# locuslab/mpc.pytorch

Hardware: AMD Instinct MI355X
Metric: LQR problem-steps/sec (batch*T/s), n_state=12 n_ctrl=4 T=50 (higher is better)
Workload: dtype f32

## Files before the change

mpc.pytorch_amd/csrc/lqr_dpp16.hip:

```cpp
#include <string>
#include "lqr_common.h"

#define MPC_DEV __device__ __forceinline__
#define DPPM " row_mask:0xf bank_mask:0xf\n"

namespace mpclqr {
namespace wv {
typedef float f32x4 __attribute__((ext_vector_type(4)));
MPC_DEV int lane() { return (int)threadIdx.x; }
MPC_DEV int problem() { return (int)blockIdx.x; }
MPC_DEV unsigned long long clock() { return (unsigned long long)clock64(); }
MPC_DEV float rcp(float x) { return __builtin_amdgcn_rcpf(x); }
MPC_DEV void pin(float &x) { asm volatile("" : "+v"(x)); }
MPC_DEV bool uniform(bool c) { return c; }
MPC_DEV int uniform(int v) { return v; }
MPC_DEV bool any(bool c) { return __ballot(c) != 0ull; }
MPC_DEV unsigned long long ballot(bool c) { return __ballot(c); }
MPC_DEV float readlane(float x, int l) { return __int_as_float(__builtin_amdgcn_readlane(__float_as_int(x), __builtin_amdgcn_readfirstlane(l))); }
MPC_DEV double readlane_f64(double x, int l)
{
    const unsigned long long b = __double_as_longlong(x);
    const int ll = __builtin_amdgcn_readfirstlane(l);
    const unsigned lo = (unsigned)__builtin_amdgcn_readlane((int)(unsigned)b, ll), hi = (unsigned)__builtin_amdgcn_readlane((int)(unsigned)(b >> 32), ll);
    return __longlong_as_double(((unsigned long long)hi << 32) | lo);
// ... 259 lines not shown
        case 62: asm volatile("v_accvgpr_read_b32 %0, a248\n v_accvgpr_read_b32 %1, a249\n v_accvgpr_read_b32 %2, a250\n v_accvgpr_read_b32 %3, a251" : "=v"(r0), "=v"(r1), "=v"(r2), "=v"(r3)); break;
        case 63: asm volatile("v_accvgpr_read_b32 %0, a252\n v_accvgpr_read_b32 %1, a253\n v_accvgpr_read_b32 %2, a254\n v_accvgpr_read_b32 %3, a255" : "=v"(r0), "=v"(r1), "=v"(r2), "=v"(r3)); break;
    }
    return f32x4{r0, r1, r2, r3};
}

MPC_DEV double dpp_f64(double x, int) { return x; }
template <int CTRL> MPC_DEV double mov_dpp_f64(double x)
{
    const unsigned long long b = __double_as_longlong(x);
    const unsigned lo = (unsigned)__builtin_amdgcn_update_dpp(0, (int)(unsigned)b, CTRL, 0xf, 0xf, true);
    const unsigned hi = (unsigned)__builtin_amdgcn_update_dpp(0, (int)(unsigned)(b >> 32), CTRL, 0xf, 0xf, true);
    return __longlong_as_double(((unsigned long long)hi << 32) | lo);
}
MPC_DEV double row_sum_f64(double x)
{
    x += mov_dpp_f64<0xB1>(x);
    x += mov_dpp_f64<0x4E>(x);
    x += mov_dpp_f64<0x141>(x);
    x += mov_dpp_f64<0x140>(x);
    return x;
}

#ifndef MPC_DPP16_NSTAGE
#define MPC_DPP16_NSTAGE 4
#endif
#ifdef MPC_KF_LDS_BYTES
#define MPC_DPP16_LDS (MPC_KF_LDS_BYTES)
#else
#define MPC_DPP16_LDS (MPC_DPP16_NSTAGE * 9216)
#endif
#ifndef MPC_KKT16_NSTAGE
#define MPC_KKT16_NSTAGE 4
#endif
#if !defined(MPC_DPP16_WITH_KKT) && !defined(MPC_DPP16_NO_KKT) && MPC_DPP16_NSTAGE == 4
#define MPC_DPP16_WITH_KKT 1
#endif
__shared__ __attribute__((aligned(16))) char g_stage16[MPC_DPP16_LDS];
typedef __attribute__((address_space(3))) void lds_void_t;
typedef __attribute__((address_space(1))) const void glb_void_t;
#ifndef MPC_DPP16_C_AUX
#define MPC_DPP16_C_AUX 2
#endif
#ifndef MPC_DPP16_FR_AUX
#define MPC_DPP16_FR_AUX 0
#endif
MPC_DEV void store_out(float *g, float v)
{
#ifdef MPC_DPP16_OUT_CACHED
    *g = v;
#else
    __builtin_nontemporal_store(v, g);
#endif
}
#ifndef MPC_KKT_LD_AUX
#define MPC_KKT_LD_AUX 0
#endif
MPC_DEV void dma16_once(const void *g, unsigned off)
{
    __builtin_amdgcn_global_load_lds((glb_void_t *)g, (lds_void_t *)(g_stage16 + off), 16, 0, MPC_KKT_LD_AUX);
}
MPC_DEV void store_f32_out(float *g, float v) { *g = v; }
typedef float f32x2 __attribute__((ext_vector_type(2)));
MPC_DEV void store_f32x2_out(float *g, float a, float b)
{
#ifdef MPC_KF_CACHED_GRADS
    *(f32x2 *)g = f32x2{a, b};
#else
    __builtin_nontemporal_store(f32x2{a, b}, (f32x2 *)g);
#endif
}
MPC_DEV void store_f32_grad(float *g, float v)
{
#ifdef MPC_KF_CACHED_GRADS
    *g = v;
#else
    __builtin_nontemporal_store(v, g);
#endif
}
typedef float f32x4_a4 __attribute__((ext_vector_type(4), aligned(4)));
MPC_DEV void store_f32x4_grad(float *g, float __attribute__((ext_vector_type(4))) v)
{
#ifdef MPC_KF_CACHED_GRADS
    *(f32x4_a4 *)g = v;
#else
    __builtin_nontemporal_store(v, (f32x4_a4 *)g);
#endif
}
MPC_DEV float swap1(float x) { return __int_as_float(__builtin_amdgcn_update_dpp(0, __float_as_int(x), 0xB1, 0xf, 0xf, true)); }
MPC_DEV void dma16_if(bool active, const void *g, unsigned off)
{
    if (active) __builtin_amdgcn_global_load_lds((glb_void_t *)g, (lds_void_t *)(g_stage16 + off), 16, 0, 0);
}
template <int G> MPC_DEV void dma_buf(bool active, const void *base, unsigned nbytes, unsigned voff, unsigned off)
{
    static_assert(G == 4, "dword gathers");
    if (active) {
        __amdgpu_buffer_rsrc_t rs = __builtin_amdgcn_make_buffer_rsrc((void *)base, (short)0, (int)nbytes, 0x00020000);
        __builtin_amdgcn_raw_ptr_buffer_load_lds(rs, (lds_void_t *)(g_stage16 + off), 4, (int)voff, 0, 0, 0);
    }
}
MPC_DEV void dma4_if(bool active, const void *g, unsigned off)
{
    if (active) __builtin_amdgcn_global_load_lds((glb_void_t *)g, (lds_void_t *)(g_stage16 + off), 4, 0, 0);
}
template <int IMM, int BIAS> MPC_DEV void dma_buf_at(const void *base_biased, unsigned nbytes_biased, unsigned voff, unsigned anchor)
{
    static_assert(IMM >= 0 && IMM < 4096, "12-bit unsigned immediate");
    __amdgpu_buffer_rsrc_t rs = __builtin_amdgcn_make_buffer_rsrc((void *)base_biased, (short)0, (int)nbytes_biased, 0x00020000);
    __builtin_amdgcn_raw_ptr_buffer_load_lds(rs, (lds_void_t *)(g_stage16 + anchor), 4, (int)voff, 0, IMM, 0);
}
template <int IMM> MPC_DEV void dma4_at_if(bool active, const void *g, unsigned anchor)
{
    if (active) __builtin_amdgcn_global_load_lds((glb_void_t *)g, (lds_void_t *)(g_stage16 + anchor), 4, IMM, 0);
}
MPC_DEV void lds_store_f32x4(unsigned off, f32x4 v) { *(f32x4 *)(g_stage16 + off) = v; }
MPC_DEV void lds_store_f32(unsigned off, float v) { *(float *)(g_stage16 + off) = v; }
MPC_DEV void lds_sync() { asm volatile("" ::: "memory"); }
enum { DMA_PLAIN = 0, DMA_C = 1, DMA_LAST = 2 };
template <int IMM, int KIND = DMA_PLAIN> MPC_DEV void dma16_at(const void *g, unsigned mid)
{
    static_assert(IMM >= -4096 && IMM < 4096, "13-bit signed immediate");
    __builtin_amdgcn_global_load_lds((glb_void_t *)g, (lds_void_t *)(g_stage16 + mid), 16, IMM,
                                     KIND == DMA_C ? MPC_DPP16_C_AUX : (KIND == DMA_LAST ? MPC_DPP16_FR_AUX : 0));
}
template <int IMM> MPC_DEV void dma16_at_if(bool active, const void *g, unsigned mid)
{
    if (active) __builtin_amdgcn_global_load_lds((glb_void_t *)g, (lds_void_t *)(g_stage16 + mid), 16, IMM, 0);
}
MPC_DEV unsigned load_uniform_u32(const unsigned *g)
{
    typedef const __attribute__((address_space(4))) unsigned const_u32_t;
    return *(const_u32_t *)(unsigned long)g;
}
MPC_DEV float lds_f32(unsigned off) { return *(const float *)(g_stage16 + off); }
MPC_DEV float bits_f32(unsigned u) { return __uint_as_float(u); }
MPC_DEV unsigned f32_bits(float f) { return __float_as_uint(f); }
MPC_DEV f32x4 lds_f32x4(unsigned off) { return *(const f32x4 *)(g_stage16 + off); }
MPC_DEV void store_f32x4(float *g, f32x4 v) { *(f32x4 *)g = v; }
template <int N> MPC_DEV void dma_wait()
{
    static_assert(N >= 0 && N < 64, "vmcnt is 6 bits on gfx9");
    asm volatile("s_waitcnt vmcnt(%0) ; counted" ::"n"(N) : "memory");
}
MPC_DEV void fence_own_stores()
{
    __builtin_amdgcn_fence(__ATOMIC_RELEASE, "workgroup");
    __builtin_amdgcn_s_waitcnt(0);
    __builtin_amdgcn_fence(__ATOMIC_ACQUIRE, "workgroup");
}
}
}

#include "lqr_dpp16_body.h"

namespace mpclqr {
namespace {

template <int MODE>
__global__ void __launch_bounds__(64, 1) lqr_step_dpp16_kernel(StepParams<float> p)
{
    dpp16::step_wave<MODE>(p);
}

#if MPC_DPP16_NSTAGE == 4 || defined(MPC_DPP16_PAD_KKT)
static_assert((int)dpp16::KfP2<false>::SLOTS * (int)dpp16::KfP2<false>::STAGE + (int)dpp16::KfP2<false>::GST <= MPC_DPP16_LDS &&
              (int)dpp16::KfP2<false>::SLOTS >= 5, "the fused KKT kernel's second ring does not fit");
static_assert((int)dpp16::KfP2<true>::SLOTS * (int)dpp16::KfP2<true>::STAGE + (int)dpp16::KfP2<true>::GST <= MPC_DPP16_LDS &&
              (int)dpp16::KfP2<true>::SLOTS >= (dpp16::PADK ? 4 : 5), "the long-horizon fused KKT kernel's second ring does not fit");
static_assert((int)dpp16::LDS_TOTAL <= MPC_DPP16_LDS, "the fused KKT kernel's sweep ring does not fit");
template <bool MASKED>
__global__ void __launch_bounds__(64, 1) lqr_kkt_fused_dpp16_kernel(StepParams<float> p, dpp16::KktFusedArgs k)
{
    dpp16::kkt_fused_wave<MASKED>(p, k);
}
template <bool MASKED>
__global__ void __launch_bounds__(64, 1) lqr_kkt_fused_long_dpp16_kernel(StepParams<float> p, dpp16::KktFusedArgs k)
{
    dpp16::kkt_fused_wave<MASKED, true>(p, k);
}

#endif

#ifdef MPC_DPP16_WITH_KKT
static_assert(MPC_KKT16_NSTAGE * 8192 <= MPC_DPP16_LDS, "the KKT kernel's ring does not fit this compilation's staging array");
__global__ void __launch_bounds__(64, 1) lqr_kkt_dpp16_kernel(StepParams<float> p, dpp16::KktArgs k)
{
    dpp16::kkt_wave(p, k);
}

#endif
}

#ifdef MPC_DPP16_WITH_KKT
bool kkt_dpp16_supported(const StepParams<float> &p, const float *dx, const float *du, const float *dl_dx,
                         const float *dC, const float *dF)
{
    auto al = [](const void *q, long st, long sb) { return ((uintptr_t)q % 16 == 0) && (st % 4 == 0) && (sb % 4 == 0); };
    if (!(p.ns == 12 && p.nc == 4 && p.T >= 1)) return false;
    if (!al(p.C, p.C_st, p.C_sb) || !al(p.c, p.c_st, p.c_sb)) return false;
    if (p.T > 1 && !al(p.F, p.F_st, p.F_sb)) return false;
    return al(p.cur_x, 0, 0) && al(p.cur_u, 0, 0) && al(dx, 0, 0) && al(du, 0, 0) && al(dl_dx, 0, 0) && al(dC, 0, 0) &&
           (p.T == 1 || al(dF, 0, 0));
}

int launch_kkt_dpp16(const StepParams<float> &p, const float *dx, const float *du, const float *dl_dx, float *dC,
                     float *dc, float *dF, float *df, float *dx_init, hipStream_t st)
{
    dpp16::KktArgs k;
    k.dx = dx; k.du = du; k.dl_dx = dl_dx; k.dC = dC; k.dc = dc; k.dF = dF; k.df = df; k.dx_init = dx_init;
    hipLaunchKernelGGL(lqr_kkt_dpp16_kernel, dim3((p.B + 3) / 4), dim3(64), 0, st, p, k);
    hipError_t e = hipGetLastError();
    if (e != hipSuccess) {
        set_last_error((std::string("lqr_kkt_dpp16_kernel: ") + hipGetErrorString(e)).c_str());
        return MPC_E_LAUNCH;
    }
    return MPC_OK;
}

#endif

#ifdef MPC_DPP16_PAD_KKT
bool kkt_fused_dpp16_pad_supported(const StepParams<float> &p, const float *ws)
{
    return p.ns >= 1 && p.ns <= 12 && p.nc >= 1 && p.nc <= 4 && p.T >= 1 && (uintptr_t)ws % 16 == 0;
}
#define MPC_KF_LAUNCH launch_kkt_fused_dpp16_pad
#elif MPC_DPP16_NSTAGE == 4
#define MPC_KF_LAUNCH launch_kkt_fused_dpp16
bool kkt_fused_dpp16_supported(const StepParams<float> &p, const float *dl_dx, const float *dl_du, const float *dC,
                               const float *dF, const float *ws)
{
    auto al = [](const void *q, long st, long sb) { return ((uintptr_t)q % 16 == 0) && (st % 4 == 0) && (sb % 4 == 0); };
    if (!(p.ns == 12 && p.nc == 4 && p.T >= 1)) return false;
    if (!al(p.C, p.C_st, p.C_sb) || !al(p.c, p.c_st, p.c_sb)) return false;
    if (p.T > 1 && !al(p.F, p.F_st, p.F_sb)) return false;
    if (p.bound_mode == MPC_BOUND_TENSOR && (!al(p.lo, 0, 0) || !al(p.hi, 0, 0))) return false;
    return al(p.cur_x, 0, 0) && al(p.cur_u, 0, 0) && al(dl_dx, 0, 0) && al(dl_du, 0, 0) && al(dC, 0, 0) && al(ws, 0, 0) &&
           (p.T == 1 || al(dF, 0, 0));
}

int64_t kkt_fused_dpp16_workspace_bytes(int T, int B)
{
    return (int64_t)T * B * (dpp16::KF_VBLK + 24 + (T > dpp16::RG_STEPS ? 64 : 0)) * 4 + 64;
}
#endif

#if MPC_DPP16_NSTAGE == 4 || defined(MPC_DPP16_PAD_KKT)
int MPC_KF_LAUNCH(const StepParams<float> &p_in, const float *dl_dx, const float *dl_du, float *dC, float *dc, float *dF,
                  float *df, float *dx_init, float *dx_out, float *du_out, float *ws, float decay, int max_ls,
                  hipStream_t st)
{
    StepParams<float> p = p_in;
    p.zero_mask = nullptr;
    p.has_delta = 0;
    if (dpp16::PADK) p.c_symmetric = 1;
    dpp16::KktFusedArgs k;
    k.dl_dx = dl_dx; k.dl_du = dl_du; k.dC = dC; k.dc = dc; k.dF = dF; k.df = df; k.dx_init = dx_init;
    k.dx_out = dx_out; k.du_out = du_out; k.vws = ws; k.decay = decay; k.max_ls = max_ls;
    const dim3 grid((p.B + 3) / 4), block(64);
    if (p.T > dpp16::RG_STEPS) {
        if (p.bound_mode != MPC_BOUND_NONE) hipLaunchKernelGGL((lqr_kkt_fused_long_dpp16_kernel<true>), grid, block, 0, st, p, k);
        else hipLaunchKernelGGL((lqr_kkt_fused_long_dpp16_kernel<false>), grid, block, 0, st, p, k);
    } else if (p.bound_mode != MPC_BOUND_NONE) hipLaunchKernelGGL((lqr_kkt_fused_dpp16_kernel<true>), grid, block, 0, st, p, k);
    else hipLaunchKernelGGL((lqr_kkt_fused_dpp16_kernel<false>), grid, block, 0, st, p, k);
    hipError_t e = hipGetLastError();
    if (e != hipSuccess) {
        set_last_error((std::string("lqr_kkt_fused_dpp16_kernel: ") + hipGetErrorString(e)).c_str());
        return MPC_E_LAUNCH;
    }
    return MPC_OK;
}

#endif

#if MPC_DPP16_NSTAGE == 4
bool dpp16_supported(const StepParams<float> &p)
{
    auto al = [](const void *q, long st, long sb) { return ((uintptr_t)q % 16 == 0) && (st % 4 == 0) && (sb % 4 == 0); };
    if (!(p.ns == 12 && p.nc == 4 && p.T >= 1 && p.max_ls >= 1 && p.max_ls <= 16)) return false;
    if (!al(p.C, p.C_st, p.C_sb) || !al(p.c, p.c_st, p.c_sb)) return false;
    if (p.T > 1 && !al(p.F, p.F_st, p.F_sb)) return false;
    if (p.f && !al(p.f, p.f_st, p.f_sb)) return false;
    if (!al(p.cur_x, 0, 0) || !al(p.cur_u, 0, 0)) return false;
    if (p.bound_mode == MPC_BOUND_TENSOR && (!al(p.lo, 0, 0) || !al(p.hi, 0, 0))) return false;
    if (p.zero_mask && (uintptr_t)p.zero_mask % 4 != 0) return false;
    return true;
}

#endif

#ifndef MPC_DPP16_PAD_KKT
#ifdef MPC_DPP16_PAD
#define MPC_DPP16_LAUNCH launch_step_dpp16_pad
bool dpp16_pad_supported(const StepParams<float> &p)
{
    return p.ns >= 1 && p.ns <= 12 && p.nc >= 1 && p.nc <= 4 && p.T >= 1 && p.max_ls >= 1 && p.max_ls <= 16 && !p.env.kind;
}
#define MPC_DPP16_TAKES(p) dpp16_pad_supported(p)
#elif MPC_DPP16_NSTAGE == 4
#define MPC_DPP16_LAUNCH launch_step_dpp16
#else
#define MPC_DPP16_LAUNCH launch_step_dpp16_ring2
bool dpp16_supported(const StepParams<float> &p);
#endif
int MPC_DPP16_LAUNCH(const StepParams<float> &p, hipStream_t st)
// ... 24 lines not shown
```

mpc.pytorch_amd/csrc/lqr_dpp16_body.h:

```cpp
#pragma once
#include <math.h>
#include "lqr_params.h"
#include "lqr_small_math.h"

#ifndef MPC_STAT
#define MPC_STAT(i)
#endif

#ifndef MPC_DEVM
#define MPC_DEVM MPC_DEV
#endif

#ifndef MPC_DPP16_NSTAGE
#define MPC_DPP16_NSTAGE 4
#endif
#ifndef MPC_DPP16_QP_WARM
#define MPC_DPP16_QP_WARM 0
#endif

#ifdef MPC_DPP16_PAD
#define MPC_DPP16_PADK 1
#else
#define MPC_DPP16_PADK 0
#endif

namespace mpclqr {
namespace dpp16 {
constexpr bool PADK = MPC_DPP16_PADK != 0;
constexpr unsigned OOB_OFF = 0x7fff0000u;
enum { PAD_BIAS = 4096 };
MPC_DEV int pad_tau(int pj, int ns, int nc) { return pj < 12 ? (pj < ns ? pj : -1) : (pj - 12 < nc ? ns + (pj - 12) : -1); }

#ifdef MPC_DPP16_PROF
struct Prof { unsigned long long acc[16]; unsigned long long last; };
#define PROF_DECL Prof prof_; for (int i_ = 0; i_ < 16; ++i_) prof_.acc[i_] = 0; prof_.last = wv::clock()
#define PROF_ARG , Prof &prof_
#define PROF_PASS , prof_
#define PROF_MARK(slot) do { asm volatile("s_waitcnt lgkmcnt(0)" ::: "memory"); const unsigned long long n_ = wv::clock(); prof_.acc[slot] += n_ - prof_.last; prof_.last = n_; } while (0)
#define PROF_MARK_ALL(slot) do { asm volatile("s_waitcnt vmcnt(0) lgkmcnt(0)" ::: "memory"); const unsigned long long n_ = wv::clock(); prof_.acc[slot] += n_ - prof_.last; prof_.last = n_; } while (0)
#else
#define PROF_DECL
#define PROF_ARG
#define PROF_PASS
#define PROF_MARK(slot)
#define PROF_MARK_ALL(slot)
#endif

typedef StepParams<float> P;
using wv::f32x4;

constexpr bool con(int MODE) { return MODE == 1 || MODE == 2; }
constexpr bool rgm(int MODE) { return MODE < 1; }

enum { RG_STEPS = 64 };
template <bool ON> struct Gains {};
MPC_DEV void gain_put(Gains<true> &, int t, f32x4 v) { wv::rg_put(t, v); }
MPC_DEV f32x4 gain_get(const Gains<true> &, int t) { return wv::rg_get(t); }
MPC_DEV void gain_put(Gains<false> &, int, f32x4) {}
MPC_DEV f32x4 gain_get(const Gains<false> &, int) { return f32x4{0.f, 0.f, 0.f, 0.f}; }
using mfma16::Sym4;
using mfma16::Ldl4;
using mfma16::ldl4;
using mfma16::ldl4_solve;
using mfma16::eclampf;
using mfma16::sel;

struct Gj4 {
    float nl[4];
    float inv[4];
};
MPC_DEV void gj4_solve(const Gj4 &g, float (&z)[4])
{
#define MPC_GJ4_APPLY(c, a) wv::fmac_bcast_settled<4 * (a)>(z[a], g.nl[c], z[c])
    MPC_GJ4_APPLY(0, 1); MPC_GJ4_APPLY(0, 2); MPC_GJ4_APPLY(0, 3);
    MPC_GJ4_APPLY(1, 0); MPC_GJ4_APPLY(1, 2); MPC_GJ4_APPLY(1, 3);
    MPC_GJ4_APPLY(2, 0); MPC_GJ4_APPLY(2, 1); MPC_GJ4_APPLY(2, 3);
    MPC_GJ4_APPLY(3, 0); MPC_GJ4_APPLY(3, 1); MPC_GJ4_APPLY(3, 2);
#undef MPC_GJ4_APPLY
#pragma unroll
    for (int a = 0; a < 4; ++a) z[a] *= g.inv[a];
}
#ifdef MPC_DPP16_QP_LDL
using QpFac4 = Ldl4;
#else
using QpFac4 = Gj4;
#endif

MPC_DEV int pnqp4_rows(const Sym4 &s, const float q[4], const float lb[4], const float ub[4], int n_iter, int j,
                       float x[4], bool fr_out[4], QpFac4 &f, bool &converged)
{
    const float reg = 1e-11f;
    const float dg[4] = {s.s00 + reg - 1.f, s.s11 + reg - 1.f, s.s22 + reg - 1.f, s.s33 + reg - 1.f};
    const bool q0 = j < 4, q1 = j < 8, q2 = j < 12;
#define MPC_QV(v0, v1, v2, v3) (q0 ? (v0) : (q1 ? (v1) : (q2 ? (v2) : (v3))))
    const float Hc[4] = {MPC_QV(s.s00, s.s01, s.s02, s.s03), MPC_QV(s.s01, s.s11, s.s12, s.s13),
                         MPC_QV(s.s02, s.s12, s.s22, s.s23), MPC_QV(s.s03, s.s13, s.s23, s.s33)};
    const float lbv = MPC_QV(lb[0], lb[1], lb[2], lb[3]), ubv = MPC_QV(ub[0], ub[1], ub[2], ub[3]);
#ifndef MPC_DPP16_QP_LDL
    const float dgv = MPC_QV(dg[0], dg[1], dg[2], dg[3]);
    const bool qd[4] = {q0, q1 && !q0, q2 && !q1, !q2};
#endif
    float xv = MPC_QV(x[0], x[1], x[2], x[3]);
    float mv = -1.f;
    float done = 0.f, conv = 0.f, full = 0.f, it_ret = (float)(n_iter - 1);
#define MPC_HV(out, v) do { out = wv::bcast<0>(v) * Hc[0]; wv::fmac_bcast_settled<4>(out, v, Hc[1]); \
                            wv::fmac_bcast_settled<8>(out, v, Hc[2]); wv::fmac_bcast_settled<12>(out, v, Hc[3]); } while (0)
    float gv;
    MPC_HV(gv, xv);
    gv += MPC_QV(q[0], q[1], q[2], q[3]);
    MPC_STAT(4);
    for (int it = 0; it < n_iter; ++it) {
        if (done == 0.f) MPC_STAT(0);
        MPC_STAT(5);
        const float r_lo = (xv == lbv) ? gv : -1.f;
        const float r_hi = (xv == ubv) ? -gv : -1.f;
        const float mnv = (fmaxf(r_lo, r_hi) > 0.f) ? 0.f : 1.f;
        const float diff = wv::ring_sum(fabsf(mnv - mv));
        const bool confirmed = (diff == 0.f) & (full != 0.f) & (done == 0.f);
        it_ret = confirmed ? (float)it : it_ret;
        conv = confirmed ? 1.f : conv;
        done = confirmed ? 1.f : done;
        if (!wv::any(done == 0.f)) break;
        if (done == 0.f) MPC_STAT(1);
        MPC_STAT(6);
#ifdef MPC_DPP16_QP_LDL
        const float mn[4] = {wv::bcast<0>(mnv), wv::bcast<4>(mnv), wv::bcast<8>(mnv), wv::bcast<12>(mnv)};
        Ldl4 fn;
        {
            const float a10 = (mn[0] * mn[1]) * s.s01, a20 = (mn[0] * mn[2]) * s.s02, a30 = (mn[0] * mn[3]) * s.s03;
            const float a21 = (mn[1] * mn[2]) * s.s12, a31 = (mn[1] * mn[3]) * s.s13, a32 = (mn[2] * mn[3]) * s.s23;
            const float a00 = fmaf(mn[0], dg[0], 1.f), a11 = fmaf(mn[1], dg[1], 1.f);
            const float a22 = fmaf(mn[2], dg[2], 1.f), a33 = fmaf(mn[3], dg[3], 1.f);
            fn.i0 = wv::rcp(a00);
            fn.l10 = a10 * fn.i0; fn.l20 = a20 * fn.i0; fn.l30 = a30 * fn.i0;
            const float d1 = fmaf(-fn.l10, a10, a11);
            fn.i1 = wv::rcp(d1);
            const float t21 = fmaf(-fn.l20, a10, a21);
            const float t31 = fmaf(-fn.l30, a10, a31);
            fn.l21 = t21 * fn.i1; fn.l31 = t31 * fn.i1;
            const float d2 = fmaf(-fn.l21, t21, fmaf(-fn.l20, a20, a22));
            fn.i2 = wv::rcp(d2);
            const float t32 = fmaf(-fn.l31, t21, fmaf(-fn.l30, a20, a32));
            fn.l32 = t32 * fn.i2;
            const float d3 = fmaf(-fn.l32, t32, fmaf(-fn.l31, t31, fmaf(-fn.l30, a30, a33)));
            fn.i3 = wv::rcp(d3);
        }
        const float rv = mnv * gv;
        float y[4];
        ldl4_solve(fn, wv::bcast<0>(rv), wv::bcast<4>(rv), wv::bcast<8>(rv), wv::bcast<12>(rv), y);
        const float dxv = -(mnv * MPC_QV(y[0], y[1], y[2], y[3]));
#else
        Gj4 fn;
        float col[4];
#define MPC_GJ4_COL(c) do { col[c] = (mnv * wv::bcast<4 * (c)>(mnv)) * Hc[c]; col[c] = qd[c] ? dgq : col[c]; } while (0)
        const float dgq = fmaf(mnv, dgv, 1.f);
        MPC_GJ4_COL(0); MPC_GJ4_COL(1); MPC_GJ4_COL(2); MPC_GJ4_COL(3);
#undef MPC_GJ4_COL
        float sol = mnv * gv, invd = 0.f;
#define MPC_GJ4_PIVOT(c) do { const float inv = wv::rcp(wv::bcast<4 * (c)>(col[c])); fn.inv[c] = inv; \
                              const float t = -(col[c] * inv); fn.nl[c] = qd[c] ? 0.f : t; invd = qd[c] ? inv : invd; } while (0)
#define MPC_GJ4_ELIM(c, m) wv::fmac_bcast_settled<4 * (m)>(col[m], col[c], fn.nl[c])
#define MPC_GJ4_RHS(c) sol = fmaf(wv::bcast<4 * (c)>(sol), fn.nl[c], sol)
        MPC_GJ4_PIVOT(0); MPC_GJ4_ELIM(0, 1); MPC_GJ4_ELIM(0, 2); MPC_GJ4_ELIM(0, 3); MPC_GJ4_RHS(0);
        MPC_GJ4_PIVOT(1); MPC_GJ4_ELIM(1, 2); MPC_GJ4_ELIM(1, 3); MPC_GJ4_RHS(1);
        MPC_GJ4_PIVOT(2); MPC_GJ4_ELIM(2, 3); MPC_GJ4_RHS(2);
        MPC_GJ4_PIVOT(3); MPC_GJ4_RHS(3);
#undef MPC_GJ4_PIVOT
#undef MPC_GJ4_ELIM
#undef MPC_GJ4_RHS
        const float dxv = -(sol * invd);
#endif
        const float nrm2 = wv::ring_sum(dxv * dxv);
        f = fn;
        mv = mnv;
        const bool small = !(nrm2 >= 1e-8f) & (done == 0.f);
        it_ret = small ? (float)it : it_ret;
        conv = small ? 1.f : conv;
        done = small ? 1.f : done;
        const float live = 1.f - done;
        const float xnv = xv + dxv;
        float xcv = eclampf(xnv, lbv, ubv);
        const float out = wv::ring_sum(fabsf(xcv - xnv));
        float dv = (xcv - xv) * live, hdv;
        MPC_HV(hdv, dv);
        const bool inside = out == 0.f;
        full = inside ? 1.f : 0.f;
        const bool test = !inside & (done == 0.f);
        if (wv::any(test)) {
            if (test) MPC_STAT(2);
            const float den = wv::ring_sum(-gv * dv), dhd = wv::ring_sum(dv * hdv);
            const float arm = fmaf(-0.5f, dhd, den) * wv::rcp(den);
            bool go = test & (arm <= 0.1f);
            if (wv::any(go)) {
                float alpha = 0.1f;
                for (int count = 1; count < 10; ++count) {
                    if (go) MPC_STAT(3);
                    const float xt = eclampf(fmaf(alpha, dxv, xv), lbv, ubv);
                    const float dt = xt - xv;
                    float hdt;
                    MPC_HV(hdt, dt);
                    const float den2 = wv::ring_sum(-gv * dt), dhd2 = wv::ring_sum(dt * hdt);
                    const float arm2 = fmaf(-0.5f, dhd2, den2) * wv::rcp(den2);
                    xcv = go ? xt : xcv;
                    dv = go ? dt : dv;
                    hdv = go ? hdt : hdv;
// ... 895 lines not shown
    if (rgm(MODE)) {
        const float mult = L.j == 12 ? alpha : dx;
        un = s.tb + wv::quad_sums(s.rec[0] * mult, s.rec[1] * mult, s.rec[2] * mult, s.rec[3] * mult, L.j);
    } else {
        un = fmaf(alpha, s.kk, s.tb);
        wv::dot_bcast12(un, dx, s.Kr);
    }
    const float pre = un;
    if (con(MODE) && s.zm) un = 0.f;
    if (MODE == 2) {
        const float dlt = p.has_delta ? p.delta_u : 3.0e38f;
        const float l = fmaxf(s.lo, s.tb - dlt), h = fminf(s.hi, s.tb + dlt);
        un = eclampf(un, l, h);
    }
    e = L.isu ? (un - pre) + (alpha - 1.f) * s.kk : 0.f;
    return un;
}

template <int MODE, bool DIRECT>
MPC_DEV float stage_price(const Lane &L, const RoStage &s, float tp, float e, float dx)
{
    if (DIRECT) {
        float sq = 0.f;
        wv::dot_bcast16(sq, tp, s.Cr);
        return tp * fmaf(0.5f, sq, s.cj);
    }
    float se = 0.f;
    wv::dot_bcast_u4(se, e, s.Sr);
    const float quad = L.isu ? e * (0.5f * se) : 0.f;
    if (!con(MODE)) return quad;
    float w = 0.f;
    wv::dot_bcast_u4(w, e, s.Mc);
    const float mult = L.j < 12 ? dx : 1.f;
    return L.j <= 12 ? fmaf(mult, w, quad) : quad;
}

template <int MODE, bool DIRECT, bool CHECK, bool PAIR = false>
MPC_DEV void rollout_step(const P &p, const Lane &L, const RoStage &s, RoState &st, int t, Feed<MODE, true, DIRECT> &feed)
{
    const bool last = (t == p.T - 1);
    feed.template part<0>();
    float e, dx;
    const float un = control_law<MODE>(p, L, s, st.xs, st.alpha, e, dx);
    const float tp = L.isu ? un : st.xs;
    feed.template part<1>();
    if (DIRECT || !rgm(MODE) || st.price_on) st.cost += stage_price<MODE, DIRECT>(L, s, tp, e, dx);
    {
        const float d = sel(L.isu, s.tb - un, 0.f);
        st.du2 = fmaf(d, d, st.du2);
    }
    if (!PADK || L.ovalid) wv::store_out(st.out, tp);
    st.out += L.ostep;
    feed.template part<2>();
    if (!DIRECT && CHECK) {
        if (t > 0) {
            float r = fabsf(st.pred - s.tb) - 1e-5f * (1.f + fabsf(s.tb));
            r = (r == r) ? r : 1.f;
            r = sel(L.isu, 0.f, r);
            st.viol = r > st.viol ? r : st.viol;
        }
        if (!last) {
            float pn = s.fj;
            wv::dot_bcast16(pn, s.tb, s.Fr);
            st.pred = pn;
        }
    }
    feed.template part<3>();
    if (!last) {
        float xn = s.fj;
        wv::dot_bcast16(xn, tp, s.Fr);
        st.xs = xn;
    }
    if (PAIR) {
        float e1, dx1;
        const float un1 = control_law<MODE>(p, L, s, st.xs1, p.ls_decay, e1, dx1);
        const float tp1 = L.isu ? un1 : st.xs1;
        st.cost1 += stage_price<MODE, DIRECT>(L, s, tp1, e1, dx1);
        {
            const float d = sel(L.isu, s.tb - un1, 0.f);
            st.du21 = fmaf(d, d, st.du21);
        }
        *st.out1 = tp1;
        st.out1 += L.ostep1;
        if (!last) {
            float xn = s.fj;
            wv::dot_bcast16(xn, tp1, s.Fr);
            st.xs1 = xn;
        }
    }
}

enum { MAX_TRIALS = 15 };
struct Trials {
    float xs[MAX_TRIALS], cost[MAX_TRIALS], alpha[MAX_TRIALS];
    float du2_last;
    float *park;
    bool park_row;
    int park_k;
};

template <int MODE, bool DIRECT>
MPC_DEV void trials_step(const P &p, const Lane &L, const RoStage &s, Trials &tr, int nt, int t)
{
    const bool last = (t == p.T - 1);
    constexpr bool PARK = MODE == 2 && !DIRECT;
#pragma unroll
    for (int k = 0; k < MAX_TRIALS; ++k) {
        if (k < nt) {
            float e, dx;
            const float un = control_law<MODE>(p, L, s, tr.xs[k], tr.alpha[k], e, dx);
            const float tp = L.isu ? un : tr.xs[k];
            tr.cost[k] += stage_price<MODE, DIRECT>(L, s, tp, e, dx);
            if (PARK && k == tr.park_k) {
                const float d = sel(L.isu, s.tb - un, 0.f);
                tr.du2_last = fmaf(d, d, tr.du2_last);
                if (tr.park_row) *tr.park = tp;
                tr.park += L.ostep1;
            }
            if (!last) {
                float xn = s.fj;
                wv::dot_bcast16(xn, tp, s.Fr);
                tr.xs[k] = xn;
            }
        }
    }
}

template <int MODE, bool MULTI, bool DIRECT, bool CHECK, bool PAIR = false>
MPC_DEV void rollout_pass(const P &p, const Lane &L, Dma &d, int wave, const Gains<rgm(MODE)> &G, RoState &st, Trials &tr, int nt, double base PROF_ARG)
{
    const int T = p.T;
    float x0 = L.isu ? 0.f : (PADK ? (L.ovalid ? p.x_init[(long)L.pb * p.ns + L.j] : 0.f) : p.x_init[(long)L.pb * 12 + L.j]);
    wv::pin(x0);
    if (MULTI) {
#pragma unroll
        for (int k = 0; k < MAX_TRIALS; ++k) { tr.xs[k] = x0; tr.cost[k] = 0.f; }
        tr.du2_last = 0.f;
        tr.park = L.scr0;
    } else {
        st.xs = x0;
        st.cost = 0.f;
        st.du2 = 0.f;
        st.pred = 0.f;
        st.out = L.out0;
        if (PAIR) {
            st.xs1 = x0;
            st.cost1 = 0.f;
            st.du21 = 0.f;
            st.out1 = L.scr0;
        }
    }
    st.price_on = MULTI || wv::any(st.alpha != 1.f);
    const bool use_zm = con(MODE) && p.zero_mask != nullptr;
    enum { NS = RollRing<MODE, DIRECT>::SLOTS, LA = NS - 1, ND = RollDma<MODE, DIRECT>::N };
    static_assert((LA - 1) * ND + 2 * LA < 64, "vmcnt is 6 bits");
    unsigned zq[NS];
#pragma unroll
    for (int i = 0; i < NS; ++i) zq[i] = 0u;
    dma_seek<MODE, true, DIRECT>(d, p, L, wave);
    pad_clear(L.lane);
#pragma unroll
    for (int i = 0; i < LA; ++i) {
        if (i < T) {
            stage_issue<MODE, true, DIRECT>(d, stage_mid<MODE, true, DIRECT>(i));
            stage_move<MODE, true, DIRECT>(d, i + 1 <= T - 2);
            if (use_zm) zq[i] = zm_pick(L, zm_fetch(p, L, i));
        }
    }
    for (int t0 = 0; t0 < T; t0 += NS) {
#pragma unroll
        for (int i = 0; i < NS; ++i) {
            const int t = t0 + i;
            if (t < T) {
                PROF_MARK(7);
                if (T - 1 - t >= LA - 1) wv::dma_wait<(LA - 1) * ND>();
                else tail_wait<(LA >= 2 ? LA - 2 : 0), ND>(T - 1 - t);
                PROF_MARK(4);
                RoStage s;
                ro_read<MODE, DIRECT>(s, p, L, t, i, zq[i]);
                if (rgm(MODE)) {
                    s.rec = gain_get(G, t);
                    if (!DIRECT && st.price_on) rg_price_terms(s, L);
                }
                PROF_MARK(5);
                const int tn = t + LA;
                ZmRaw zr = {{0u, 0u, 0u, 0u}};
                if (use_zm && tn < T) zr = zm_fetch(p, L, tn);
                Feed<MODE, true, DIRECT> feed = {d, stage_mid<MODE, true, DIRECT>((i + LA) % NS), tn < T, tn + 1 <= T - 2};
                PROF_MARK(6);
                if (MULTI) {
                    feed.template part<0>(); feed.template part<1>(); feed.template part<2>(); feed.template part<3>();
                    trials_step<MODE, DIRECT>(p, L, s, tr, nt, t);
                } else {
                    rollout_step<MODE, DIRECT, CHECK, PAIR>(p, L, s, st, t, feed);
                }
                if (use_zm) zq[(i + LA) % NS] = zm_pick(L, zr);
            }
        }
    }
    wv::dma_wait<0>();
    if (MULTI) {
#pragma unroll
        for (int k = 0; k < MAX_TRIALS; ++k)
            if (k < nt) tr.cost[k] = (float)(base + (double)wv::row_sum(tr.cost[k]));
        tr.du2_last = wv::row_sum(tr.du2_last);
    } else {
        st.cost = (float)(base + (double)wv::row_sum(st.cost));
        st.du2 = wv::row_sum(st.du2);
        if (PAIR) {
            st.cost1 = (float)(base + (double)wv::row_sum(st.cost1));
            st.du21 = wv::row_sum(st.du21);
        }
    }
}

MPC_DEV Lane lane_as_slot(const Lane &L, int ps, const P &p, int wave)
{
    Lane X = L;
    const int dp = ps - L.p;
    const int pb = 4 * wave + ps < p.B ? 4 * wave + ps : p.B - 1;
    X.p = ps;
    X.pb = pb;
#pragma unroll
    for (int q = 0; q < 4; ++q) X.aFq[q] += dp * 768;
    X.aRec += dp * 256; X.aRecA += dp * 256; X.aRecF += dp * 256;
    X.aKrow += dp * 256; X.aMcol += dp * 256; X.aGcol += dp * 256; X.aFm += dp * 256;
#pragma unroll
    for (int b = 0; b < 4; ++b) X.aS[b] += dp * 256;
    X.scr0 = p.Kk + (long)p.T * p.B * 128 + (long)pb * 16 + L.j;
    return X;
}

template <int MODE, bool DIRECT, bool CHECK>
MPC_DEV void line_search(const P &p, const Lane &L, Dma &d, int wave, const Gains<rgm(MODE)> &G, RoState &rs, float old_cost, double base, float &full2 PROF_ARG)
{
    Trials tr;
    rs.alpha = 1.f;
    bool worse0 = false;
    bool copy_parked = false;
    if (MODE == 2 && !DIRECT && p.max_ls >= 2) {
        rollout_pass<MODE, false, DIRECT, CHECK, true>(p, L, d, wave, G, rs, tr, 0, base PROF_PASS);
        full2 = rs.du2;
        worse0 = rs.cost > old_cost;
        if (!wv::any(worse0)) return;
        const bool worse1 = worse0 && rs.cost1 > old_cost && p.max_ls > 2;
        if (worse0) {
            rs.alpha = p.ls_decay;
            rs.cost = rs.cost1;
            rs.du2 = rs.du21;
        }
        if (wv::any(worse1)) {
            const int nt = p.max_ls - 2;
            bool ended_on_last = false;
            const unsigned long long wm = wv::ballot(worse1 && L.j == 0);
            const int n_w = (int)__builtin_popcountll(wm);
            const bool shared = n_w == 1 && nt >= 4;
            const int ps1 = (int)(__builtin_ctzll(wm | (1ull << 63)) >> 4);
            const int nt_row = shared ? (nt + 3) / 4 : nt;
            const int r_last = shared ? (nt - 1) / nt_row : 0;
            if (shared) MPC_STAT(7); else MPC_STAT(8);
            {
                const int ps = ps1;
                const Lane X = lane_as_slot(L, shared ? ps : L.p, p, wave);
                const int idx0 = shared ? L.p * nt_row : 0;
                float a = p.ls_decay;
                for (int i = 0; i <= (idx0 < nt - 1 ? idx0 : nt - 1); ++i) a *= p.ls_decay;
#pragma unroll
                for (int k = 0; k < MAX_TRIALS; ++k) {
                    tr.alpha[k] = a;
                    if (idx0 + k + 1 <= nt - 1) a *= p.ls_decay;
                }
                tr.park_k = shared ? (L.p == r_last ? (nt - 1) - r_last * nt_row : -1) : nt - 1;
                tr.park_row = shared || worse1;
                const double base_s = shared ? wv::readlane_f64(base, 16 * ps) : base;
                const float old_s = shared ? wv::readlane(old_cost, 16 * ps) : old_cost;
                rollout_pass<MODE, true, DIRECT, CHECK>(p, X, d, wave, G, rs, tr, nt_row, base_s PROF_PASS);
                float acc = 0.f, cacc = 0.f, du2_l = tr.du2_last;
                int kacc = 0;
                bool found = false;
                if (shared) {
#pragma unroll
                    for (int r = 0; r < 4; ++r) {
#pragma unroll
                        for (int k = 0; k < MAX_TRIALS; ++k) {
                            if (k < nt_row && r * nt_row + k < nt && !found) {
                                acc = wv::readlane(tr.alpha[k], 16 * r);
                                cacc = wv::readlane(tr.cost[k], 16 * r);
                                kacc = r * nt_row + k;
                                if (!(cacc > old_s)) found = true;
                            }
                        }
                    }
                    du2_l = wv::readlane(tr.du2_last, 16 * r_last);
                } else {
#pragma unroll
                    for (int k = 0; k < MAX_TRIALS; ++k) {
                        if (k < nt && !found) {
                            acc = tr.alpha[k];
                            cacc = tr.cost[k];
                            kacc = k;
                            if (!(tr.cost[k] > old_cost)) found = true;
                        }
                    }
                }
                if (shared ? L.p == ps : worse1) {
                    rs.alpha = acc;
                    ended_on_last = kacc == nt - 1;
                    if (ended_on_last) { rs.cost = cacc; rs.du2 = du2_l; }
                }
            }
            if (wv::any(worse1 && !ended_on_last)) {
                rollout_pass<MODE, false, DIRECT, CHECK>(p, L, d, wave, G, rs, tr, 0, base PROF_PASS);
                return;
            }
        }
        copy_parked = true;
    }
    if (copy_parked) {
        PROF_MARK_ALL(9);
        wv::fence_own_stores();
        enum { COPY_N = 16 };
        const float *src = L.scr0;
        float *dst = L.out0;
        const int T = p.T;
        for (int t0 = 0; t0 < T; t0 += COPY_N) {
            float v[COPY_N];
#pragma unroll
            for (int i = 0; i < COPY_N; ++i) {
                const int t = t0 + i < T ? t0 + i : T - 1;
                v[i] = src[(long)t * L.ostep1];
            }
#pragma unroll
            for (int i = 0; i < COPY_N; ++i) {
                const int t = t0 + i < T ? t0 + i : T - 1;
                if (worse0 && (!PADK || L.ovalid)) wv::store_out(dst + (long)t * L.ostep, v[i]);
            }
        }
        PROF_MARK_ALL(12);
        return;
    }
#pragma unroll 1
    for (int phase = 0; phase < 3; ++phase) {
        rollout_pass<MODE, false, DIRECT, CHECK>(p, L, d, wave, G, rs, tr, 0, base PROF_PASS);
        if (phase == 0) {
            full2 = rs.du2;
            worse0 = rs.cost > old_cost && p.max_ls > 1;
            if (!wv::any(worse0)) break;
            if (worse0) rs.alpha = p.ls_decay;
        } else if (phase == 1) {
            const bool worse1 = worse0 && rs.cost > old_cost && p.max_ls > 2;
            if (!wv::any(worse1)) break;
            const int nt = p.max_ls - 2;
            float a = p.ls_decay;
#pragma unroll
            for (int k = 0; k < MAX_TRIALS; ++k) { a *= p.ls_decay; tr.alpha[k] = a; }
            rollout_pass<MODE, true, DIRECT, CHECK>(p, L, d, wave, G, rs, tr, nt, base PROF_PASS);
            if (worse1) {
                float acc = tr.alpha[0];
                bool found = false;
#pragma unroll
                for (int k = 0; k < MAX_TRIALS; ++k) {
                    if (k < nt && !found) {
                        acc = tr.alpha[k];
                        if (!(tr.cost[k] > old_cost)) found = true;
                    }
                }
                rs.alpha = acc;
            }
        }
    }
}

template <int MODE>
MPC_DEV void step_wave(const P &p)
{
    const int lane = wv::lane();
    const int wave = wv::problem();
    if (4 * wave >= p.B) return;
    Lane L;
    lane_init(L, lane, wave, p.B, !p.c_symmetric);
    L.out0 = L.isu ? p.new_u + (long)L.pb * 4 + L.a : p.new_x + (long)L.pb * 12 + L.j;
    L.ostep = L.isu ? (long)p.B * 4 : (long)p.B * 12;
    if (PADK) {
        L.ovalid = L.isu ? L.a < p.nc : L.j < p.ns;
#pragma unroll
        for (int a = 0; a < 4; ++a) L.padd[a] = (L.j == 12 + a && a >= p.nc) ? 1.f : 0.f;
        L.out0 = L.isu ? p.new_u + (long)L.pb * p.nc + (L.ovalid ? L.a : 0) : p.new_x + (long)L.pb * p.ns + (L.ovalid ? L.j : 0);
        L.ostep = L.isu ? (long)p.B * p.nc : (long)p.B * p.ns;
    }
    L.scr0 = p.Kk + (long)p.T * p.B * 128 + (long)L.pb * 16 + L.j;
    L.ostep1 = (long)p.B * 16;
    const int T = p.T;
    Dma d;
    Gains<rgm(MODE)> G;
    PROF_DECL;

    SwState ss;
#pragma unroll
    for (int i = 0; i < 12; ++i) ss.Vc[i] = 0.f;
    ss.vv = 0.f;
    ss.oc = 0.0;
    ss.w0 = 0.0;
    ss.warm = 0;
    ss.qp_total = 0;
    ss.status = 0;
    ss.asym = 0.f;
    ss.cmax = 0.f;
    ss.kprev[0] = ss.kprev[1] = ss.kprev[2] = ss.kprev[3] = 0.f;
    ss.rec_step = (long)p.B * 64;
    ss.rec = p.Kk + ((long)(T - 1) * p.B + L.pb) * 64 + 4 * L.j;
    ss.rec2_step = (long)p.B * 4;
    ss.rec2 = p.Kk + (long)T * p.B * 64 + ((long)(T - 1) * p.B + L.pb) * 4;
    {
        unsigned zq[NSTAGE] = {};
        dma_seek<MODE, false, false>(d, p, L, wave);
        pad_clear(L.lane);
#pragma unroll
        for (int i = 0; i < AHEAD; ++i) {
            const int ti = T - 1 - i;
            if (ti >= 0) {
                stage_issue<MODE, false, false>(d, stage_mid<MODE, false, false>(i));
                stage_move<MODE, false, false>(d, ti <= T - 2);
                if (MODE == 1) zq[i] = zm_pick(L, zm_fetch(p, L, ti));
            }
        }
        for (int k0 = 0; k0 < T; k0 += NSTAGE) {
#pragma unroll
            for (int i = 0; i < NSTAGE; ++i) {
                const int t = T - 1 - (k0 + i);
                if (t >= 0) {
                    PROF_MARK(3);
                    if (t >= AHEAD - 1) wv::dma_wait<(AHEAD - 1) * DMA_SWEEP>();
                    else wv::dma_wait<0>();
                    PROF_MARK(0);
                    SwStage s;
                    sw_read<MODE>(s, p, L, t, i, zq[i], ss.asym, ss.cmax);
                    PROF_MARK(1);
                    ZmRaw zr = {{0u, 0u, 0u, 0u}};
                    if (MODE == 1 && t >= AHEAD) zr = zm_fetch(p, L, t - AHEAD);
                    Feed<MODE, false, false> feed = {d, stage_mid<MODE, false, false>((i + AHEAD) % NSTAGE), t >= AHEAD, true};
                    PROF_MARK(2);
                    sweep_step<MODE>(p, L, s, ss, t, feed, G PROF_PASS);
                    if (MODE == 1) zq[(i + AHEAD) % NSTAGE] = zm_pick(L, zr);
                }
            }
        }
        wv::dma_wait<0>();
    }
    PROF_MARK_ALL(8);
    const double old_cost_d = wv::row_sum_f64(ss.oc);
    const float old_cost = (float)old_cost_d;
    if (!p.c_symmetric) ss.status |= MPC_ST_C_TESTED | (wv::row_max(ss.asym) > 1e-5f * wv::row_max(ss.cmax) ? (int)MPC_ST_C_ASYMMETRIC : 0);

    if (p.sweep_only) {
        if (L.j == 0) {
            if (p.old_costs) p.old_costs[L.pb] = old_cost;
            if (p.qp_iters) p.qp_iters[L.pb] = ss.qp_total;
            if (p.status) p.status[L.pb] = ss.status;
        }
        return;
    }
    wv::fence_own_stores();

    RoState rs;
    rs.viol = 0.f;
    float full2 = 0.f;
    if (p.on_dynamics) {
        line_search<MODE, false, false>(p, L, d, wave, G, rs, old_cost, old_cost_d + ss.w0, full2 PROF_PASS);
    } else {
        line_search<MODE, false, true>(p, L, d, wave, G, rs, old_cost, old_cost_d + ss.w0, full2 PROF_PASS);
        const bool off = wv::row_sum(rs.viol > 0.f ? 1.f : 0.f) > 0.f;
        const bool broken = off || (MODE == 2 && (ss.status & MPC_ST_PNQP_UNCONVERGED) != 0);
        if (wv::any(broken)) line_search<MODE, true, false>(p, L, d, wave, G, rs, old_cost, 0.0, full2 PROF_PASS);
        if (off) ss.status |= MPC_ST_NOMINAL_OFF_DYNAMICS;
    }
#ifdef MPC_DPP16_PROF
    PROF_MARK_ALL(9);
    if (p.K != nullptr && lane == 0)
        for (int i_ = 0; i_ < 16; ++i_) p.K[(long)wave * 16 + i_] = (float)prof_.acc[i_];
#endif
    int status = ss.status;
    if (!(rs.cost == rs.cost) || fabsf(rs.cost) > 3e38f) status |= MPC_ST_NONFINITE;
    if (L.j == 0) {
        const int b = L.pb;
        if (p.costs) p.costs[b] = rs.cost;
        if (p.old_costs) p.old_costs[b] = old_cost;
        if (p.full_du_norm) p.full_du_norm[b] = sqrtf(full2);
        if (p.alpha_du_norm) p.alpha_du_norm[b] = sqrtf(rs.du2);
        if (p.alphas) p.alphas[b] = rs.alpha;
        if (p.qp_iters) p.qp_iters[b] = ss.qp_total;
        if (p.status) p.status[b] = status;
    }
}


struct KktArgs {
    const float *dx, *du, *dl_dx;
    float *dC, *dc, *dF, *df, *dx_init;
};

#ifndef MPC_KKT16_NSTAGE
#define MPC_KKT16_NSTAGE 4
#endif
enum { K_c = 0, K_tau = 64, K_dtau = 128, K_rx = 192, KKT_STAGE = 8192, DMA_KKT = 8, KKT_NSTAGE = MPC_KKT16_NSTAGE,
       KKT_AHEAD = KKT_NSTAGE - 1 };

struct KktDma {
    const char *c_ptr[4];
    const char *f_ptr[3];
    const char *r_ptr;
    long c_step, f_step, r_step;
    bool r_active;
};

MPC_DEV void kkt_dma_init(KktDma &d, const P &p, const KktArgs &k, const Lane &L, int wave)
{
    const long B = p.B;
#pragma unroll
    for (int q = 0; q < 4; ++q) {
        const int pbk = 4 * wave + q < p.B ? 4 * wave + q : p.B - 1;
        d.c_ptr[q] = (const char *)(p.C + (long)pbk * p.C_sb) + 16 * src_granule_C(L.lane, 0);
    }
    d.c_step = 4 * p.C_st;
#pragma unroll
    for (int q = 0; q < 3; ++q) {
        const int G = 64 * q + L.lane;
        const int slot = G / 48, gi = G - 48 * slot;
        const int pbk = 4 * wave + slot < p.B ? 4 * wave + slot : p.B - 1;
        d.f_ptr[q] = p.T > 1 ? (const char *)(p.F + (long)pbk * p.F_sb) + 16 * src_granule_cols(gi, slot) : (const char *)p.C;
    }
    d.f_step = 4 * p.F_st;
    const int gi = L.lane & 15;
    const long pb = L.pb;
    d.r_active = gi < 15;
    const char *q = (const char *)p.c;
    long st = 0;
    if (gi < 4) { q = (const char *)(p.c + pb * p.c_sb + 4 * gi); st = 4 * p.c_st; }
    else if (gi < 7) { q = (const char *)(p.cur_x + pb * 12 + 4 * (gi - 4)); st = 4 * B * 12; }
    else if (gi == 7) { q = (const char *)(p.cur_u + pb * 4); st = 4 * B * 4; }
    else if (gi < 11) { q = (const char *)(k.dx + pb * 12 + 4 * (gi - 8)); st = 4 * B * 12; }
    else if (gi == 11) { q = (const char *)(k.du + pb * 4); st = 4 * B * 4; }
    else if (gi < 15) { q = (const char *)(k.dl_dx + pb * 12 + 4 * (gi - 12)); st = 4 * B * 12; }
    d.r_ptr = q;
    d.r_step = st;
}

MPC_DEV void kkt_stage_issue(const P &p, const KktDma &d, int t, int slot)
{
    const unsigned base = (unsigned)slot * KKT_STAGE;
    const long tl = t;
    const long tf = t < p.T - 1 ? t : (p.T > 1 ? p.T - 2 : 0);
#pragma unroll
    for (int q = 0; q < 4; ++q) wv::dma16_once(d.c_ptr[q] + tl * d.c_step, base + SC + 1024 * q);
#pragma unroll
    for (int q = 0; q < 3; ++q) wv::dma16_once(d.f_ptr[q] + (p.T > 1 ? tf * d.f_step : 0), base + SF + 1024 * q);
    wv::dma16_if(d.r_active, d.r_ptr + tl * d.r_step, base + SR);
}

MPC_DEV void kkt_wave(const P &p, const KktArgs &k)
{
    const int lane = wv::lane();
    const int wave = wv::problem();
    if (4 * wave >= p.B) return;
    Lane L;
    lane_init(L, lane, wave, p.B, false);
    const int T = p.T;
    KktDma d;
    kkt_dma_init(d, p, k, L, wave);
    float lam = 0.f, dlam = 0.f;
#pragma unroll
    for (int i = 0; i < KKT_AHEAD; ++i) kkt_stage_issue(p, d, T - 1 - i >= 0 ? T - 1 - i : 0, i);
    for (int k0 = 0; k0 < T; k0 += KKT_NSTAGE) {
#pragma unroll
        for (int i = 0; i < KKT_NSTAGE; ++i) {
            const int t = T - 1 - (k0 + i);
            if (t >= 0) {
                wv::dma_wait<(KKT_AHEAD - 1) * DMA_KKT>();
                const unsigned base = (unsigned)i * KKT_STAGE;
                float Cr[16], Fc[12];
#pragma unroll
                for (int q = 0; q < 4; ++q) {
                    const f32x4 v = wv::lds_f32x4(base + L.aCq[q]);
                    Cr[4 * q] = v[0]; Cr[4 * q + 1] = v[1]; Cr[4 * q + 2] = v[2]; Cr[4 * q + 3] = v[3];
                }
                const bool have = t < T - 1;
                if (have) {
#pragma unroll
                    for (int m = 0; m < 12; ++m) Fc[m] = wv::lds_f32(base + ((m & 1) ? L.aFo : L.aFe) + 64 * m);
                } else {
#pragma unroll
                    for (int m = 0; m < 12; ++m) Fc[m] = 0.f;
                }
                const float cj = wv::lds_f32(base + L.aRec + K_c);
                const float tj = wv::lds_f32(base + L.aRec + K_tau);
                const float dj = wv::lds_f32(base + L.aRec + K_dtau);
                const float rj = wv::lds_f32(base + SR + L.p * 256 + K_rx + 4 * (L.j < 12 ? L.j : 11));
// ... 608 lines not shown
```

Before: 2.248 billion.

## Software-pipeline LDS stage reads one step ahead in sweep and rollout loops

Adds a double-buffered register stage so the LDS reads for step t±1 are issued before computing step t, in both the backward sweep and the forward rollout, for unconstrained non-padded modes. The DMA lookahead is restructured so the whole ring is in flight (LA = NSTAGE) while waits use one fewer slot, and an explicit LDS drain waitcnt is inserted per step. The aim is to hide LDS read latency behind the previous step's math. The cost is extra register pressure, and the rollout ring is capped at four slots in regularised modes.

```diff
diff --git a/mpc.pytorch_amd/csrc/lqr_dpp16.hip b/mpc.pytorch_amd/csrc/lqr_dpp16.hip
--- a/mpc.pytorch_amd/csrc/lqr_dpp16.hip
+++ b/mpc.pytorch_amd/csrc/lqr_dpp16.hip
@@ -435,6 +435,7 @@
 }
 }
 
+#define MPC_LDS_DRAIN() __builtin_amdgcn_s_waitcnt(0xc07f)
 #include "lqr_dpp16_body.h"
 
 namespace mpclqr {
diff --git a/mpc.pytorch_amd/csrc/lqr_dpp16_body.h b/mpc.pytorch_amd/csrc/lqr_dpp16_body.h
--- a/mpc.pytorch_amd/csrc/lqr_dpp16_body.h
+++ b/mpc.pytorch_amd/csrc/lqr_dpp16_body.h
@@ -16,6 +16,12 @@
 #endif
 #ifndef MPC_DPP16_QP_WARM
 #define MPC_DPP16_QP_WARM 0
+#endif
+#ifndef MPC_DPP16_PREFETCH
+#define MPC_DPP16_PREFETCH 3
+#endif
+#ifndef MPC_LDS_DRAIN
+#define MPC_LDS_DRAIN()
 #endif
 
 #ifdef MPC_DPP16_PAD
@@ -51,6 +57,8 @@
 
 constexpr bool con(int MODE) { return MODE == 1 || MODE == 2; }
 constexpr bool rgm(int MODE) { return MODE < 1; }
+enum { PF_SWEEP = 1, PF_ROLL = 2 };
+constexpr bool pf(int MODE, int HALF) { return !PADK && !con(MODE) && ((MPC_DPP16_PREFETCH) & HALF) != 0; }
 
 enum { RG_STEPS = 64 };
 template <bool ON> struct Gains {};
@@ -1252,9 +1260,12 @@
     }
     st.price_on = MULTI || wv::any(st.alpha != 1.f);
     const bool use_zm = con(MODE) && p.zero_mask != nullptr;
-    enum { NS = RollRing<MODE, DIRECT>::SLOTS, LA = NS - 1, ND = RollDma<MODE, DIRECT>::N };
-    static_assert((LA - 1) * ND + 2 * LA < 64, "vmcnt is 6 bits");
+    constexpr bool PF = pf(MODE, PF_ROLL) && !DIRECT;
+    enum { NSE = RollRing<MODE, DIRECT>::SLOTS & ~1, NS = PF ? (rgm(MODE) && NSE > 4 ? 4 : NSE) : (int)RollRing<MODE, DIRECT>::SLOTS,
+           LA = PF ? NS : NS - 1, LW = NS - 1, ND = RollDma<MODE, DIRECT>::N };
+    static_assert(NS >= 2 && (LW - 1) * ND + 2 * LA < 64, "vmcnt is 6 bits");
     unsigned zq[NS];
+    RoStage ro[2];
 #pragma unroll
     for (int i = 0; i < NS; ++i) zq[i] = 0u;
     dma_seek<MODE, true, DIRECT>(d, p, L, wave);
@@ -1267,27 +1278,43 @@
             if (use_zm) zq[i] = zm_pick(L, zm_fetch(p, L, i));
         }
     }
+    if (PF) {
+        if (T >= LA) wv::dma_wait<(LA - 1) * ND>();
+        else wv::dma_wait<0>();
+        ro_read<MODE, DIRECT>(ro[0], p, L, 0, 0, 0u);
+        if (rgm(MODE)) ro[0].rec = gain_get(G, 0);
+    }
     for (int t0 = 0; t0 < T; t0 += NS) {
 #pragma unroll
         for (int i = 0; i < NS; ++i) {
             const int t = t0 + i;
             if (t < T) {
+                const int ts = PF ? t + 1 : t;
+                RoStage &s = ro[PF ? i & 1 : 0];
                 PROF_MARK(7);
-                if (T - 1 - t >= LA - 1) wv::dma_wait<(LA - 1) * ND>();
-                else tail_wait<(LA >= 2 ? LA - 2 : 0), ND>(T - 1 - t);
+                if (PF) MPC_LDS_DRAIN();
+                if (ts < T) {
+                    if (T - 1 - ts >= LW - 1) wv::dma_wait<(LW - 1) * ND>();
+                    else tail_wait<(LW >= 2 ? LW - 2 : 0), ND>(T - 1 - ts);
+                }
                 PROF_MARK(4);
-                RoStage s;
-                ro_read<MODE, DIRECT>(s, p, L, t, i, zq[i]);
-                if (rgm(MODE)) {
-                    s.rec = gain_get(G, t);
-                    if (!DIRECT && st.price_on) rg_price_terms(s, L);
-                }
-                PROF_MARK(5);
+                if (PF) {
+                    if (ts < T) {
+                        RoStage &sn = ro[(i + 1) & 1];
+                        ro_read<MODE, DIRECT>(sn, p, L, ts, (i + 1) % NS, 0u);
+                        if (rgm(MODE)) sn.rec = gain_get(G, ts);
+                    }
+                } else {
+                    ro_read<MODE, DIRECT>(s, p, L, t, i, zq[i]);
+                    if (rgm(MODE)) s.rec = gain_get(G, t);
+                }
+                if (rgm(MODE) && !DIRECT && st.price_on) rg_price_terms(s, L);
+                if (!PF) { PROF_MARK(5); }
                 const int tn = t + LA;
                 ZmRaw zr = {{0u, 0u, 0u, 0u}};
                 if (use_zm && tn < T) zr = zm_fetch(p, L, tn);
                 Feed<MODE, true, DIRECT> feed = {d, stage_mid<MODE, true, DIRECT>((i + LA) % NS), tn < T, tn + 1 <= T - 2};
-                PROF_MARK(6);
+                if (!PF) { PROF_MARK(6); }
                 if (MULTI) {
                     feed.template part<0>(); feed.template part<1>(); feed.template part<2>(); feed.template part<3>();
                     trials_step<MODE, DIRECT>(p, L, s, tr, nt, t);
@@ -1512,11 +1539,15 @@
     ss.rec2_step = (long)p.B * 4;
     ss.rec2 = p.Kk + (long)T * p.B * 64 + ((long)(T - 1) * p.B + L.pb) * 4;
     {
+        constexpr bool PF = pf(MODE, PF_SWEEP);
+        enum { LA = PF ? (int)NSTAGE : (int)AHEAD, LW = PF ? (int)NSTAGE - 1 : (int)AHEAD };
+        static_assert(!PF || NSTAGE % 2 == 0, "two register sets alternate through the unrolled trips");
         unsigned zq[NSTAGE] = {};
+        SwStage sw[2];
         dma_seek<MODE, false, false>(d, p, L, wave);
         pad_clear(L.lane);
 #pragma unroll
-        for (int i = 0; i < AHEAD; ++i) {
+        for (int i = 0; i < LA; ++i) {
             const int ti = T - 1 - i;
             if (ti >= 0) {
                 stage_issue<MODE, false, false>(d, stage_mid<MODE, false, false>(i));
@@ -1524,24 +1555,37 @@
                 if (MODE == 1) zq[i] = zm_pick(L, zm_fetch(p, L, ti));
             }
         }
+        if (PF) {
+            if (T >= LA) wv::dma_wait<(LA - 1) * DMA_SWEEP>();
+            else wv::dma_wait<0>();
+            sw_read<MODE>(sw[0], p, L, T - 1, 0, 0u, ss.asym, ss.cmax);
+        }
         for (int k0 = 0; k0 < T; k0 += NSTAGE) {
 #pragma unroll
             for (int i = 0; i < NSTAGE; ++i) {
                 const int t = T - 1 - (k0 + i);
                 if (t >= 0) {
+                    const int ts = PF ? t - 1 : t;
+                    SwStage &s = sw[PF ? i & 1 : 0];
                     PROF_MARK(3);
-                    if (t >= AHEAD - 1) wv::dma_wait<(AHEAD - 1) * DMA_SWEEP>();
-                    else wv::dma_wait<0>();
+                    if (PF) MPC_LDS_DRAIN();
+                    if (ts >= 0) {
+                        if (ts >= LW - 1) wv::dma_wait<(LW - 1) * DMA_SWEEP>();
+                        else wv::dma_wait<0>();
+                    }
                     PROF_MARK(0);
-                    SwStage s;
-                    sw_read<MODE>(s, p, L, t, i, zq[i], ss.asym, ss.cmax);
-                    PROF_MARK(1);
+                    if (PF) {
+                        if (ts >= 0) sw_read<MODE>(sw[(i + 1) & 1], p, L, ts, (i + 1) % NSTAGE, 0u, ss.asym, ss.cmax);
+                    } else {
+                        sw_read<MODE>(s, p, L, t, i, zq[i], ss.asym, ss.cmax);
+                        PROF_MARK(1);
+                    }
                     ZmRaw zr = {{0u, 0u, 0u, 0u}};
-                    if (MODE == 1 && t >= AHEAD) zr = zm_fetch(p, L, t - AHEAD);
-                    Feed<MODE, false, false> feed = {d, stage_mid<MODE, false, false>((i + AHEAD) % NSTAGE), t >= AHEAD, true};
-                    PROF_MARK(2);
+                    if (MODE == 1 && t >= LA) zr = zm_fetch(p, L, t - LA);
+                    Feed<MODE, false, false> feed = {d, stage_mid<MODE, false, false>((i + LA) % NSTAGE), t >= LA, true};
+                    if (!PF) { PROF_MARK(2); }
                     sweep_step<MODE>(p, L, s, ss, t, feed, G PROF_PASS);
-                    if (MODE == 1) zq[(i + AHEAD) % NSTAGE] = zm_pick(L, zr);
+                    if (MODE == 1) zq[(i + LA) % NSTAGE] = zm_pick(L, zr);
                 }
             }
         }
```

New measurement: 2.257 billion (median of 6 runs). About the same (+0.4%).
